# fulliu/lc

Measured on AMD Instinct MI355X. Metric: poses/sec (cov-loss fwd+bwd + weighted PnP), B=256 N=64, 1/2/4/8 MI355X, higher is better.
Workload: dtype f64; 1 GPU; configs[1]: synthetic B=256 N=64 2D-3D correspondences per GPU, HIP weighted-PnP + cov-loss; global_batch=256, n_points=64, launch=graph_region, launch_agreed_by_all_ranks=True

## Files before the change

### lc_amd/csrc/lc_common.h

```cpp
#pragma once
#include <hip/hip_runtime.h>

namespace lc {

#ifndef LC_NT_GRAD_STORES
#define LC_NT_GRAD_STORES 1
#endif
typedef float lc_v4f_t __attribute__((ext_vector_type(4)));
__device__ __forceinline__ void store_stream4(float* q, float a, float b, float c, float d) {
#if LC_NT_GRAD_STORES
    lc_v4f_t r = {a, b, c, d};
    __builtin_nontemporal_store(r, reinterpret_cast<lc_v4f_t*>(q));
#else
    *reinterpret_cast<float4*>(q) = make_float4(a, b, c, d);
#endif
}


constexpr int kWave = 64;

constexpr int kDppQuadXor1 = 0xB1;
constexpr int kDppQuadXor2 = 0x4E;
constexpr int kDppIdentity = 0xE4;
constexpr int kDppRowMirror = 0x140;
constexpr int kDppHalfMirror = 0x141;

template <int CTRL, int BANK_MASK = 0xF>
__device__ __forceinline__ double dpp_mov_f64(double old, double src) {
    const int lo = __builtin_amdgcn_update_dpp(__double2loint(old), __double2loint(src), CTRL, 0xF, BANK_MASK, false);
    const int hi = __builtin_amdgcn_update_dpp(__double2hiint(old), __double2hiint(src), CTRL, 0xF, BANK_MASK, false);
    return __hiloint2double(hi, lo);
}

__device__ __forceinline__ double shfl_f64(double v, int src) {
    const int lo = __shfl(__double2loint(v), src, kWave), hi = __shfl(__double2hiint(v), src, kWave);
    return __hiloint2double(hi, lo);
}

__device__ __forceinline__ double swap32_add(double a, double b) {
    const auto lo = __builtin_amdgcn_permlane32_swap(__double2loint(a), __double2loint(b), false, false);
    const auto hi = __builtin_amdgcn_permlane32_swap(__double2hiint(a), __double2hiint(b), false, false);
    return __hiloint2double(hi[0], lo[0]) + __hiloint2double(hi[1], lo[1]);
}
__device__ __forceinline__ double swap16_add(double a, double b) {
    const auto lo = __builtin_amdgcn_permlane16_swap(__double2loint(a), __double2loint(b), false, false);
    const auto hi = __builtin_amdgcn_permlane16_swap(__double2hiint(a), __double2hiint(b), false, false);
    return __hiloint2double(hi[0], lo[0]) + __hiloint2double(hi[1], lo[1]);
}

template <int CTRL, int BANK_UP>
__device__ __forceinline__ double dpp_exchange_add(double lo, double hi) {
    constexpr int BANK_DOWN = 0xF & ~BANK_UP;
    const double keep = dpp_mov_f64<kDppIdentity, BANK_UP>(lo, hi);
    double recv = dpp_mov_f64<CTRL, BANK_UP>(lo, hi);
    recv = dpp_mov_f64<CTRL, BANK_DOWN>(recv, lo);
    return keep + recv;
}

template <int K>
__device__ __forceinline__ void wave_allreduce(double (&v)[K]) {
#pragma unroll
    for (int i = 0; i < K; ++i) {
        double x = v[i];
        x += dpp_mov_f64<kDppQuadXor1>(x, x);
        x += dpp_mov_f64<kDppQuadXor2>(x, x);
        x += dpp_mov_f64<kDppHalfMirror>(x, x);
        x += dpp_mov_f64<kDppRowMirror>(x, x);
        x = swap16_add(x, x);
        x = swap32_add(x, x);
        v[i] = x;
    }
}

template <int K>
__device__ __forceinline__ void wave_reduce_scatter16(double (&v)[K], int ) {
    static_assert(K % 16 == 0, "K must be a multiple of 16");
    constexpr int R = K / 16;
#pragma unroll
    for (int i = 0; i < K / 2; ++i) v[i] = swap32_add(v[i], v[i + K / 2]);
#pragma unroll
    for (int i = 0; i < K / 4; ++i) v[i] = swap16_add(v[i], v[i + K / 4]);
#pragma unroll
    for (int i = 0; i < K / 8; ++i) v[i] = dpp_exchange_add<kDppRowMirror, 0xC>(v[i], v[i + K / 8]);
#pragma unroll
    for (int i = 0; i < K / 16; ++i) v[i] = dpp_exchange_add<kDppHalfMirror, 0xA>(v[i], v[i + K / 16]);
#pragma unroll
    for (int i = 0; i < R; ++i) {
        v[i] += dpp_mov_f64<kDppQuadXor2>(v[i], v[i]);
        v[i] += dpp_mov_f64<kDppQuadXor1>(v[i], v[i]);
    }
}

__device__ __forceinline__ int scatter16_base(int lane, int R) {
    return R * (((lane >> 5) & 1) * 8 + ((lane >> 4) & 1) * 4 + ((lane >> 3) & 1) * 2 + ((lane >> 2) & 1));
}

__device__ __forceinline__ double fast_rcp(double x) {
    const double y = __builtin_amdgcn_rcp(x);
    const double e = __builtin_fma(-x, y, 1.0);
    return __builtin_fma(y, e, y);
}

__device__ __forceinline__ void fast_sqrt_rsqrt(double x, double& s, double& rs) {
    const double r0 = __builtin_amdgcn_rsq(x);
    const double g = x * r0, h = 0.5 * r0;
    const double rr = __builtin_fma(-h, g, 0.5);
    const double g1 = __builtin_fma(g, rr, g), h1 = __builtin_fma(h, rr, h);
    s = x == 0.0 ? 0.0 : g1;
    rs = x == 0.0 ? r0 : 2.0 * h1;
}
__device__ __forceinline__ double fast_sqrt(double x) {
    double s, rs;
    fast_sqrt_rsqrt(x, s, rs);
    return s;
}

template <int NW>
constexpr int sum_bcast_lds_doubles(int K) { return K * 68 * NW + K; }

#ifndef LC_WAVE_SYNC
#define LC_WAVE_SYNC 0
#endif
__device__ __forceinline__ void wave_sync() {
    __builtin_amdgcn_fence(__ATOMIC_RELEASE, "wavefront");
    __builtin_amdgcn_wave_barrier();
    __builtin_amdgcn_fence(__ATOMIC_ACQUIRE, "wavefront");
}

template <class T>
__device__ __forceinline__ void xcd_store(T* q, T v) { __hip_atomic_store(q, v, __ATOMIC_RELAXED, __HIP_MEMORY_SCOPE_AGENT); }
template <class T>
__device__ __forceinline__ T xcd_load(const T* q) { return __hip_atomic_load(q, __ATOMIC_RELAXED, __HIP_MEMORY_SCOPE_AGENT); }
__device__ __forceinline__ void xcd_stores_done() { asm volatile("s_waitcnt vmcnt(0)" ::: "memory"); }

constexpr int kArrivalShards = 16, kArrivalStride = 32;
constexpr int kArrivalWords = (1 + kArrivalShards) * kArrivalStride;
__device__ __forceinline__ bool arrive_is_last(unsigned* words, unsigned block, unsigned blocks) {
    const unsigned shards = blocks < (unsigned)kArrivalShards ? blocks : (unsigned)kArrivalShards;
    const unsigned g = block % shards, members = (blocks - g + shards - 1) / shards;
    if (__hip_atomic_fetch_add(words + (1 + g) * kArrivalStride, 1u, __ATOMIC_RELAXED, __HIP_MEMORY_SCOPE_AGENT) != members - 1) return false;
    return __hip_atomic_fetch_add(words, 1u, __ATOMIC_RELAXED, __HIP_MEMORY_SCOPE_AGENT) == shards - 1;
}
__device__ __forceinline__ void arrival_reset(unsigned* words, int tid) {
    if (tid <= kArrivalShards) xcd_store(words + tid * kArrivalStride, 0u);
}

template <int NW>
__device__ __forceinline__ void block_sum_sync() {
    if constexpr (NW == 1 && !LC_WAVE_SYNC) wave_sync();
    else __syncthreads();
}

template <int NW>
__device__ __forceinline__ int block_sum_open(int tid) {
    block_sum_sync<NW>();
    return tid + 2 * (tid >> 5);
}
template <int NW>
__device__ __forceinline__ void block_sum_put(double* lds, int pos, int k, double v) { lds[k * (68 * NW) + pos] = v; }

template <int K, int NW>
__device__ __forceinline__ void block_sum_close(double (&v)[K], double* lds, int tid);

template <int K, int NW>
__device__ __forceinline__ void block_sum_bcast_lds(double (&v)[K], double* lds, int tid) {
    const int pos = block_sum_open<NW>(tid);
#pragma unroll
    for (int k = 0; k < K; ++k) block_sum_put<NW>(lds, pos, k, v[k]);
    block_sum_close<K, NW>(v, lds, tid);
}

template <int K, int NW>
__device__ __forceinline__ double* block_sum_totals(double* lds) { return lds + K * (68 * NW); }

template <int K, int NW>
__device__ __forceinline__ void block_sum_reduce(double* lds, int tid) {
    static_assert(K <= 32 && (NW == 1 || NW == 4), "unsupported shape");
    constexpr int LD = 68 * NW, S = 2 * NW;
    block_sum_sync<NW>();
    double s = 0;
    if (tid < K * S) {
        const double2* row = reinterpret_cast<const double2*>(lds + (tid / S) * LD + 34 * (tid % S));
        double2 a[8];
#pragma unroll
        for (int i = 0; i < 8; ++i) a[i] = row[i];
#pragma unroll
        for (int i = 0; i < 8; ++i) {
            const double2 t = row[8 + i];
            a[i].x += t.x;
            a[i].y += t.y;
        }
#pragma unroll
        for (int st = 4; st >= 1; st >>= 1) {
#pragma unroll
            for (int i = 0; i < st; ++i) { a[i].x += a[i + st].x; a[i].y += a[i + st].y; }
        }
        s = a[0].x + a[0].y;
    }
    s += dpp_mov_f64<kDppQuadXor1>(s, s);
    if constexpr (NW == 4) {
        s += dpp_mov_f64<kDppQuadXor2>(s, s);
        s += dpp_mov_f64<kDppHalfMirror>(s, s);
    }
    double* tot = lds + K * LD;
    if (tid < K * S && (tid % S) == 0) tot[tid / S] = s;
    block_sum_sync<NW>();
}

template <int K, int NW>
__device__ __forceinline__ void block_sum_close(double (&v)[K], double* lds, int tid) {
    block_sum_reduce<K, NW>(lds, tid);
    const double* tot = block_sum_totals<K, NW>(lds);
#pragma unroll
    for (int k = 0; k < K; ++k) v[k] = tot[k];
}

#ifndef LC_WIDE_SUM_REGS
#define LC_WIDE_SUM_REGS 1
#endif
template <int K>
__device__ __forceinline__ void block_sum_waves4(double (&v)[K], double* lds, int tid, int& phase) {
    static_assert(K <= 32, "one reduce-scatter of 32");
    const int lane = tid & 63, wave = tid >> 6;
    double w[32];
#pragma unroll
    for (int k = 0; k < 32; ++k) w[k] = k < K ? v[k] : 0.0;
    wave_reduce_scatter16<32>(w, lane);
    double* part = lds;
    double* tot = lds + 128 + 32 * phase;
    phase ^= 1;
    if ((lane & 3) == 0) *reinterpret_cast<double2*>(part + 32 * wave + scatter16_base(lane, 2)) = make_double2(w[0], w[1]);
    __syncthreads();
    if (tid < 32) tot[tid] = ((part[tid] + part[32 + tid]) + part[64 + tid]) + part[96 + tid];
    __syncthreads();
#pragma unroll
    for (int k = 0; k < K; ++k) v[k] = tot[k];
}

constexpr int kSplitMaxParts = 8;
#ifndef LC_SPLIT_WAIT_US
#define LC_SPLIT_WAIT_US 2000
#endif
constexpr unsigned long long kSplitWaitTicks = 100ull * LC_SPLIT_WAIT_US;
__device__ __forceinline__ bool split_wait_expired(int polls, unsigned long long& t0) {
    if ((polls & 15) != 15) return false;
    const unsigned long long now = __builtin_amdgcn_s_memrealtime();
    if (t0 == 0) { t0 = now; return false; }
    return now - t0 > kSplitWaitTicks;
}
constexpr int kSplitRowWords = 64;
constexpr size_t kSplitPoseBytes = 2 * kSplitMaxParts * kSplitRowWords * sizeof(unsigned long long) + 128;
constexpr int kSplitLdsDoubles = 128 + 64 + 2;
constexpr int kSplitSerialLdsDoubles = 128 + 32 * kSplitMaxParts + 32;
struct SplitSum {
    unsigned long long* exch;
    unsigned* epoch;
    int G, part;
    unsigned base;
    unsigned seq;
    bool timed_out;
};
__device__ __forceinline__ unsigned* split_tail(void* region, size_t region_bytes) {
    return reinterpret_cast<unsigned*>(static_cast<char*>(region) + region_bytes - 128);
}
__device__ __forceinline__ SplitSum split_sum_enter(void* pose_region, int G, int part) {
    unsigned* epoch = split_tail(pose_region, kSplitPoseBytes);
    return SplitSum{reinterpret_cast<unsigned long long*>(pose_region), epoch, G, part, xcd_load(epoch), 0u, false};
}
__device__ __forceinline__ void split_sum_leave(const SplitSum& sx) {
    if (sx.timed_out) xcd_store(sx.epoch + 1, 1u);
    else if (sx.part == 0 && sx.seq > 0) xcd_store(sx.epoch, sx.base + sx.seq);
}
__device__ __forceinline__ bool split_rescue_enter(void* region, size_t region_bytes, bool redo, int tid, int threads) {
    unsigned* tail = split_tail(region, region_bytes);
    const bool dirty = xcd_load(tail + 1) != 0u;
    if (!dirty && !redo) return false;
    __syncthreads();
    if (dirty) {
        unsigned long long* w = static_cast<unsigned long long*>(region);
        for (size_t i = tid; i < (region_bytes - 128) / 8; i += threads) xcd_store(w + i, 0ull);
        if (tid < 2) xcd_store(tail + tid, 0u);
    }
    if (redo && tid == 0) xcd_store(tail + 2, xcd_load(tail + 2) + 1u);
    return redo;
}

template <int K>
__device__ __forceinline__ void block_sum_split(double (&v)[K], double* lds, int tid, int& phase, SplitSum& sx) {
    static_assert(K <= 32, "one reduce-scatter of 32");
    const int lane = tid & 63, wave = tid >> 6;
    double w[32];
#pragma unroll
    for (int k = 0; k < 32; ++k) w[k] = k < K ? v[k] : 0.0;
    wave_reduce_scatter16<32>(w, lane);
    double* part = lds;
    double* tot = lds + 128 + 32 * phase;
    int* arrived_ok = reinterpret_cast<int*>(lds + 192);
    phase ^= 1;
    if (sx.timed_out) {
#pragma unroll
        for (int k = 0; k < K; ++k) v[k] = 0.0;
        return;
    }
    if ((lane & 3) == 0) *reinterpret_cast<double2*>(part + 32 * wave + scatter16_base(lane, 2)) = make_double2(w[0], w[1]);
    __syncthreads();
    if (tid < 32) {
        const unsigned long long ticket = (unsigned long long)(sx.base + sx.seq + 1u) << 32;
        unsigned long long* rows = sx.exch + (size_t)(sx.seq & 1u) * (kSplitMaxParts * kSplitRowWords) + 2 * tid;
        {
            const unsigned long long bits = __builtin_bit_cast(unsigned long long, ((part[tid] + part[32 + tid]) + part[64 + tid]) + part[96 + tid]);
            unsigned long long* mine = rows + sx.part * kSplitRowWords;
            xcd_store(mine, ticket | (bits & 0xFFFFFFFFull));
            xcd_store(mine + 1, ticket | (bits >> 32));
        }
        unsigned long long lo[kSplitMaxParts], hi[kSplitMaxParts];
        bool ok = true;
        unsigned long long t0 = 0;
        for (int polls = 0;; ++polls) {
#pragma unroll
            for (int g = 0; g < kSplitMaxParts; ++g)
                if (g < sx.G) {
                    lo[g] = xcd_load(rows + g * kSplitRowWords);
                    hi[g] = xcd_load(rows + g * kSplitRowWords + 1);
                }
            unsigned long long late = 0;
#pragma unroll
            for (int g = 0; g < kSplitMaxParts; ++g)
                if (g < sx.G) late |= ((lo[g] ^ ticket) | (hi[g] ^ ticket)) >> 32;
            if (late == 0) break;
            if (split_wait_expired(polls, t0)) { ok = false; break; }
            __builtin_amdgcn_s_sleep(1);
        }
        double s = 0.0;
#pragma unroll
        for (int g = 0; g < kSplitMaxParts; ++g)
            if (g < sx.G) s += __builtin_bit_cast(double, (hi[g] << 32) | (lo[g] & 0xFFFFFFFFull));
        tot[tid] = s;
        if (!ok) *arrived_ok = 0;
    }
    __syncthreads();
    if (!*arrived_ok) sx.timed_out = true;
#pragma unroll
    for (int k = 0; k < K; ++k) v[k] = tot[k];
    ++sx.seq;
}

template <int K>
__device__ __forceinline__ void block_sum_parts_serial(double (&v)[K], double* lds, int tid, int g, int G) {
    static_assert(K <= 32, "one reduce-scatter of 32");
    const int lane = tid & 63, wave = tid >> 6;
    double w[32];
#pragma unroll
    for (int k = 0; k < 32; ++k) w[k] = k < K ? v[k] : 0.0;
    wave_reduce_scatter16<32>(w, lane);
    double* part = lds;
    double* rows = lds + 128;
    double* tot = lds + 128 + 32 * kSplitMaxParts;
    if ((lane & 3) == 0) *reinterpret_cast<double2*>(part + 32 * wave + scatter16_base(lane, 2)) = make_double2(w[0], w[1]);
    __syncthreads();
    if (tid < 32) {
        rows[32 * g + tid] = ((part[tid] + part[32 + tid]) + part[64 + tid]) + part[96 + tid];
        if (g == G - 1) {
            double s = 0.0;
            for (int h = 0; h < G; ++h) s += rows[32 * h + tid];
            tot[tid] = s;
        }
    }
    __syncthreads();
    if (g == G - 1) {
#pragma unroll
        for (int k = 0; k < K; ++k) v[k] = tot[k];
    }
}

#ifndef LC_HORNER_ASM
#define LC_HORNER_ASM 1
#endif
__device__ __forceinline__ double horner_step(double p, double z, double c) {
#if LC_HORNER_ASM
    double r;
    asm("v_fma_f64 %0, %1, %2, %3" : "=v"(r) : "v"(p), "v"(z), "v"(c));
    return r;
#else
    return __builtin_fma(p, z, c);
#endif
}

__device__ __forceinline__ void sincos_small(double x, double& s, double& c) {
    if (!(x < 1.0e4)) {
        sincos(x, &s, &c);
        return;
    }
    const double kf = __builtin_rint(x * 0.63661977236758134308);
    const int q = (int)kf;
    double r = __builtin_fma(-kf, 1.57079632673412561417e+00, x);
    r = __builtin_fma(-kf, 6.07710050650619224932e-11, r);
    r = __builtin_fma(-kf, 2.02226624879595063154e-21, r);
    const double z = r * r;
    double ps = horner_step(1.58969099521155010221e-10, z, -2.50507602534068634195e-08);
    ps = horner_step(ps, z, 2.75573137070700676789e-06);
    ps = horner_step(ps, z, -1.98412698298579493134e-04);
    ps = horner_step(ps, z, 8.33333333332248946124e-03);
    ps = horner_step(ps, z, -1.66666666666666324348e-01);
    const double sr = __builtin_fma(ps * z, r, r);
    double pc = horner_step(-1.13596475577881948265e-11, z, 2.08757232129817482790e-09);
    pc = horner_step(pc, z, -2.75573143513906633035e-07);
    pc = horner_step(pc, z, 2.48015872894767294178e-05);
    pc = horner_step(pc, z, -1.38888888888741095749e-03);
    pc = horner_step(pc, z, 4.16666666666666019037e-02);
    const double cr = __builtin_fma(pc * z, z, __builtin_fma(-0.5, z, 1.0));
    const double ss = (q & 1) ? cr : sr, cc = (q & 1) ? sr : cr;
    s = (q & 2) ? -ss : ss;
    c = ((q + 1) & 2) ? -cc : cc;
}

__device__ __forceinline__ double atan_ratio_pos(double s, double c) {
    const bool swap = s > c;
    const double a = swap ? c : s, b = swap ? s : c;
    double t = a * fast_rcp(b);
#pragma unroll
    for (int k = 0; k < 2; ++k) {
        const double h = fast_sqrt(__builtin_fma(t, t, 1.0));
        t = t * fast_rcp(1.0 + h);
    }
    const double w = t * t;
    double p = horner_step(-1.0 / 21.0, w, 1.0 / 19.0);
    p = horner_step(p, w, -1.0 / 17.0);
    p = horner_step(p, w, 1.0 / 15.0);
    p = horner_step(p, w, -1.0 / 13.0);
    p = horner_step(p, w, 1.0 / 11.0);
    p = horner_step(p, w, -1.0 / 9.0);
    p = horner_step(p, w, 1.0 / 7.0);
    p = horner_step(p, w, -1.0 / 5.0);
    p = horner_step(p, w, 1.0 / 3.0);
    const double at = 4.0 * __builtin_fma(-(p * w), t, t);
    return swap ? 1.57079632679489661923 - at : at;
}

__device__ __forceinline__ bool uniform(bool c) { return __builtin_amdgcn_ballot_w64(c) != 0ull; }

__host__ __device__ constexpr int tri6(int i, int j) { return i * 6 - (i * (i - 1)) / 2 + (j - i); }

}
```

### lc_amd/csrc/lc_pnp_body.h

```cpp
#pragma once
#include <cfloat>

#include "lc_common.h"
#include "lc_kernels.h"

#ifdef LC_STAMPS
#define LC_PSTAMP_DECL unsigned long long pst_[8] = {0, 0, 0, 0, 0, 0, 0, 0}, pt0_ = 0, pt1_ = 0
#define LC_PSTAMP_BEGIN()                                                                 \
    do {                                                                                  \
        __builtin_amdgcn_sched_barrier(0);                                                \
        asm volatile("s_memtime %0\n\ts_waitcnt lgkmcnt(0)" : "=s"(pt0_)::"memory");      \
        __builtin_amdgcn_sched_barrier(0);                                                \
    } while (0)
#define LC_PSTAMP(i)                                                                      \
    do {                                                                                  \
        __builtin_amdgcn_sched_barrier(0);                                                \
        asm volatile("s_memtime %0\n\ts_waitcnt lgkmcnt(0)" : "=s"(pt1_)::"memory");      \
        __builtin_amdgcn_sched_barrier(0);                                                \
        pst_[i] += pt1_ - pt0_;                                                           \
        pt0_ = pt1_;                                                                      \
    } while (0)
#else
#define LC_PSTAMP_DECL
#define LC_PSTAMP_BEGIN() do {} while (0)
#define LC_PSTAMP(i) do {} while (0)
#endif

#ifndef LC_WIDE_REG_SUM_REGS
#define LC_WIDE_REG_SUM_REGS 1
#endif
#ifndef LC_PNP_STREAM_SUM
#define LC_PNP_STREAM_SUM 1
#endif

namespace lc {
namespace pnp {

template <int NW>
constexpr int kPnpLdsDoubles = sum_bcast_lds_doubles<NW>(28);

struct Point {
    double X[3];
    double u, v;
    double a, b, c;
};

struct Rot {
    double R[9];
    double Jr[9];
};

__device__ __forceinline__ void make_rot(const double aa[3], Rot& o) {
    const double x = aa[0], y = aa[1], z = aa[2];
    const double th2 = x * x + y * y + z * z;
    const bool small = !(th2 > DBL_EPSILON);
    double th, ith;
    fast_sqrt_rsqrt(th2, th, ith);
    double s, c;
    sincos_small(th, s, c);
    const double ith2 = ith * ith;
    const double A = small ? 1.0 : s * ith;
    const double B = small ? 0.0 : (1.0 - c) * ith2;
    const double C = small ? 0.0 : (th - s) * ith2 * ith;
    const double cd = small ? 1.0 : c;
    o.R[0] = cd + B * x * x;    o.R[1] = B * x * y - A * z; o.R[2] = B * x * z + A * y;
    o.R[3] = B * x * y + A * z; o.R[4] = cd + B * y * y;    o.R[5] = B * y * z - A * x;
    o.R[6] = B * x * z - A * y; o.R[7] = B * y * z + A * x; o.R[8] = cd + B * z * z;
    const double d = 1.0 - C * th2;
    o.Jr[0] = d + C * x * x;     o.Jr[1] = C * x * y + B * z; o.Jr[2] = C * x * z - B * y;
    o.Jr[3] = C * x * y - B * z; o.Jr[4] = d + C * y * y;     o.Jr[5] = C * y * z + B * x;
    o.Jr[6] = C * x * z + B * y; o.Jr[7] = C * y * z - B * x; o.Jr[8] = d + C * z * z;
}

template <bool FIRST, bool STREAM = false, int NW = 1>
__device__ __forceinline__ void accumulate_point(const Point& pt, const Rot& rt, const double t[3], const double k[6],
                                                 const double (&sc)[6], double (&acc)[28], double* lds = nullptr, int pos = 0) {
    double rx[3], q[3];
#pragma unroll
    for (int d = 0; d < 3; ++d) {
        rx[d] = rt.R[3 * d] * pt.X[0] + rt.R[3 * d + 1] * pt.X[1] + rt.R[3 * d + 2] * pt.X[2];
        q[d] = rx[d] + t[d];
    }
    const double iz = fast_rcp(q[2]);
    const double up = (q[0] * k[0] + q[1] * k[1]) * iz, vp = (q[0] * k[3] + q[1] * k[4]) * iz;
    const double du = up - pt.u, dv = vp - pt.v;
    const double r[2] = {du * pt.a + dv * pt.b, dv * pt.c};
    const double dup[3] = {k[0] * iz, k[1] * iz, -up * iz};
    const double dvp[3] = {k[3] * iz, k[4] * iz, -vp * iz};
    double J[2][6];
#pragma unroll
    for (int m = 0; m < 3; ++m) {
        J[0][3 + m] = pt.a * dup[m] + pt.b * dvp[m];
        J[1][3 + m] = pt.c * dvp[m];
    }
#pragma unroll
    for (int rr = 0; rr < 2; ++rr) {
        double cr[3];
        cr[0] = rx[1] * J[rr][5] - rx[2] * J[rr][4];
        cr[1] = rx[2] * J[rr][3] - rx[0] * J[rr][5];
        cr[2] = rx[0] * J[rr][4] - rx[1] * J[rr][3];
#pragma unroll
        for (int m = 0; m < 3; ++m) J[rr][m] = (rt.Jr[3 * m] * cr[0] + rt.Jr[3 * m + 1] * cr[1] + rt.Jr[3 * m + 2] * cr[2]) * sc[m];
#pragma unroll
        for (int m = 0; m < 3; ++m) J[rr][3 + m] *= sc[3 + m];
    }
#pragma unroll
    for (int i = 0; i < 6; ++i) {
#pragma unroll
        for (int j = i; j < 6; ++j) {
            const double v = __builtin_fma(J[0][i], J[0][j], J[1][i] * J[1][j]);
            if constexpr (STREAM) block_sum_put<NW>(lds, pos, tri6(i, j), v);
            else acc[tri6(i, j)] = FIRST ? v : acc[tri6(i, j)] + v;
        }
        const double gi = __builtin_fma(J[0][i], r[0], J[1][i] * r[1]);
        if constexpr (STREAM) block_sum_put<NW>(lds, pos, 21 + i, gi);
        else acc[21 + i] = FIRST ? gi : acc[21 + i] + gi;
    }
    const double ss = __builtin_fma(r[0], r[0], r[1] * r[1]);
    if constexpr (STREAM) block_sum_put<NW>(lds, pos, 27, ss);
    else acc[27] = FIRST ? ss : acc[27] + ss;
}

__device__ __forceinline__ bool ldlt_solve6(const double (&A)[21], const double (&dg)[6], const double (&rhs)[6], double (&y)[6]) {
    double L[6][6], Ld[6][6], id[6];
    bool ok = true;
#pragma unroll
    for (int j = 0; j < 6; ++j) {
        double dj = A[tri6(j, j)] + dg[j];
#pragma unroll
        for (int k = 0; k < j; ++k) dj -= L[j][k] * Ld[j][k];
        ok = ok && (dj > 0) && (dj < DBL_MAX);
        id[j] = fast_rcp(dj);
#pragma unroll
        for (int i = j + 1; i < 6; ++i) {
            double v = A[tri6(j, i)];
#pragma unroll
            for (int k = 0; k < j; ++k) v -= L[i][k] * Ld[j][k];
            Ld[i][j] = v;
            L[i][j] = v * id[j];
        }
    }
    double z[6];
#pragma unroll
    for (int i = 0; i < 6; ++i) {
        double v = rhs[i];
#pragma unroll
        for (int k = 0; k < i; ++k) v -= L[i][k] * z[k];
        z[i] = v;
    }
#pragma unroll
    for (int i = 5; i >= 0; --i) {
        double v = z[i] * id[i];
#pragma unroll
        for (int k = i + 1; k < 6; ++k) v -= L[k][i] * y[k];
        y[i] = v;
    }
    return ok;
}

struct RawPoint {
    float X[3];
    float2 u;
    float a, b, c;
};
__device__ __forceinline__ float nan_to_num(float f) { return f != f ? 0.f : fminf(fmaxf(f, -FLT_MAX), FLT_MAX); }

template <bool OPTS = false>
__device__ __forceinline__ RawPoint load_raw_point(const PnpParams& p, size_t base, int n) {
    RawPoint o;
    const float* X = p.pts3d + (base + n) * 3;
    o.u = *reinterpret_cast<const float2*>(p.pts2d + (base + n) * 2);
    o.X[0] = X[0]; o.X[1] = X[1]; o.X[2] = X[2];
    if (OPTS && p.weight_mask) {
        const float m = p.weight_mask[base + n] ? 1.f : 0.f;
        o.a = m; o.b = 0.f; o.c = m;
    } else if (p.sqrtL) {
        const float4 L = *reinterpret_cast<const float4*>(p.sqrtL + (base + n) * 4);
        o.a = L.x; o.b = L.z; o.c = L.w;
    } else {
        const float2 L = *reinterpret_cast<const float2*>(p.sqrt_diag + (base + n) * 2);
        o.a = L.x; o.b = 0.f; o.c = L.y;
    }
    if constexpr (OPTS) {
        if (p.options & kPnpWeightsAreStd) { o.a = 1.f / (o.a * o.a); o.c = 1.f / (o.c * o.c); }
        if (p.options & kPnpNanToNum) {
            o.u.x = nan_to_num(o.u.x); o.u.y = nan_to_num(o.u.y);
            o.X[0] = nan_to_num(o.X[0]); o.X[1] = nan_to_num(o.X[1]); o.X[2] = nan_to_num(o.X[2]);
            o.a = nan_to_num(o.a); o.b = nan_to_num(o.b); o.c = nan_to_num(o.c);
        }
        if (p.options & kPnpWeightsAreIcov) { o.a = sqrtf(o.a); o.c = sqrtf(o.c); }
    }
    return o;
}
__device__ __forceinline__ Point to_point(const RawPoint& r, const double cam[6]) {
    Point o;
    o.X[0] = r.X[0]; o.X[1] = r.X[1]; o.X[2] = r.X[2];
    o.u = (double)r.u.x - cam[2];
    o.v = (double)r.u.y - cam[5];
    o.a = r.a; o.b = r.b; o.c = r.c;
    return o;
}
template <bool OPTS = false>
__device__ __forceinline__ Point load_point(const PnpParams& p, size_t base, int n, const double cam[6]) {
    return to_point(load_raw_point<OPTS>(p, base, n), cam);
}

__device__ __forceinline__ double max_abs6(const double (&v)[6]) {
    double m = 0;
#pragma unroll
    for (int j = 0; j < 6; ++j) m = fmax(m, fabs(v[j]));
    return m;
}
__device__ __forceinline__ double norm6(const double (&v)[6]) {
    double m = 0;
#pragma unroll
    for (int j = 0; j < 6; ++j) m += v[j] * v[j];
    return fast_sqrt(m);
}

template <bool REG, int NW = 1, bool TRACE = false, bool OPTS = false, int PPT = 0, bool TAIL = false, int SPLIT = 0>
__device__ __forceinline__ void solve_pose(const PnpParams& p, int b, int lane, double* bc, bool store = true, float* handoff = nullptr,
                                           const float* start_override = nullptr, [[maybe_unused]] SplitSum* sx = nullptr) {
    constexpr int kThreads = kWave * NW;
    static_assert(SPLIT != 1 || (NW == 4 && !REG && PPT > 0 && !TRACE), "the split form is the four-wave cached-prefix solve");
    static_assert(SPLIT != 2 || (NW == 4 && !REG && PPT == 0 && !TRACE), "the rescue form walks memory, part by part");
    const int slot = SPLIT == 1 ? lane + kThreads * sx->part : lane;
    const int stride = SPLIT == 1 ? kThreads * sx->G : kThreads;
#ifdef LC_TRACE_CLOCK
    const unsigned long long t_start_ = __builtin_amdgcn_s_memtime();
#endif
    LC_PSTAMP_DECL;
    LC_PSTAMP_BEGIN();
    const int n = p.counts ? p.counts[b] : p.Nmax;
    const int bk = (OPTS && p.pose_mod > 0) ? b % p.pose_mod : b;
    const float* st_in = start_override ? start_override : (p.start ? p.start + 7 * (size_t)bk : p.states + 7 * (size_t)b);
    const bool filter = OPTS && (p.options & kPnpNanToNum);
    auto fin = [&](float f) { return filter ? nan_to_num(f) : f; };
    if (n < 3) {
        if (lane == 0 && store) {
            p.rets[b] = 1;
            p.result_tr[b] = 1.f;
            if (p.iters) p.iters[b] = 0;
        }
        if (lane < 7) {
            const float v = fin(st_in[lane]);
            if (store && (p.start || start_override || filter)) p.states[7 * (size_t)b + lane] = v;
            if (handoff) handoff[lane] = v;
        }
        return;
    }
    const size_t base = (size_t)b * p.Nmax;
    const bool active = lane < n;
    RawPoint raw;
    if constexpr (REG) raw = load_raw_point<OPTS>(p, base, active ? lane : 0);
    [[maybe_unused]] RawPoint rawc[PPT > 0 ? PPT : 1];
    if constexpr (!REG && PPT > 0) {
#pragma unroll
        for (int k = 0; k < PPT; ++k)
            if (slot + k * stride < n) rawc[k] = load_raw_point<OPTS>(p, base, slot + k * stride);
    }
    double cam[6];
    {
        const float* Kp = p.K + 9 * (size_t)bk;
#pragma unroll
        for (int i = 0; i < 6; ++i) cam[i] = fin(Kp[i]);
    }
    double x[6];
    {
        float stf[7];
#pragma unroll
        for (int i = 0; i < 7; ++i) stf[i] = st_in[i];
        asm volatile("" : "+v"(stf[0]), "+v"(stf[1]), "+v"(stf[2]), "+v"(stf[3]), "+v"(stf[4]), "+v"(stf[5]), "+v"(stf[6]));
        const double q0 = fin(stf[0]), q1 = fin(stf[1]), q2 = fin(stf[2]), q3 = fin(stf[3]);
        const double s2 = q1 * q1 + q2 * q2 + q3 * q3;
        double kk = 2.0;
        if (s2 > 0.0) {
            const double s = fast_sqrt(s2);
            const double half = atan_ratio_pos(s, fabs(q0));
            const double two_theta = 2.0 * ((q0 < 0.0) ? -half : half);
            kk = two_theta / s;
        }
        x[0] = q1 * kk; x[1] = q2 * kk; x[2] = q3 * kk;
        x[3] = fin(stf[4]); x[4] = fin(stf[5]); x[5] = fin(stf[6]);
    }
    LC_PSTAMP(0);
    Point rp;
    if constexpr (REG) {
        rp = to_point(raw, cam);
        if (!active) { rp.a = 0.0; rp.b = 0.0; rp.c = 0.0; }
    }

    [[maybe_unused]] int sum_phase = 0;
    auto evaluate = [&](const double (&xe)[6], const double (&sc)[6], double (&H)[21], double (&g)[6], double& cost) -> bool {
        LC_PSTAMP(1);
        Rot rt;
        make_rot(xe, rt);
        LC_PSTAMP(2);
        const double t[3] = {xe[3], xe[4], xe[5]};
        double acc[28];
        if constexpr (REG && LC_PNP_STREAM_SUM && !(NW == 4 && LC_WIDE_REG_SUM_REGS)) {
            const int pos = block_sum_open<NW>(lane);
            accumulate_point<true, true, NW>(rp, rt, t, cam, sc, acc, bc, pos);
            LC_PSTAMP(3);
            block_sum_close<28, NW>(acc, bc, lane);
        } else if constexpr (REG) {
            accumulate_point<true>(rp, rt, t, cam, sc, acc);
            LC_PSTAMP(3);
            if constexpr (NW == 4 && LC_WIDE_SUM_REGS) block_sum_waves4<28>(acc, bc, lane, sum_phase);
            else block_sum_bcast_lds<28, NW>(acc, bc, lane);
        } else {
#pragma unroll
            for (int i = 0; i < 28; ++i) acc[i] = 0;
            if constexpr (PPT > 0) {
#pragma unroll
                for (int k = 0; k < PPT; ++k)
                    if (slot + k * stride < n) accumulate_point<false>(to_point(rawc[k], cam), rt, t, cam, sc, acc);
                if constexpr (TAIL)
                    for (int i = slot + PPT * stride; i < n; i += stride) accumulate_point<false>(load_point<OPTS>(p, base, i, cam), rt, t, cam, sc, acc);
            } else if constexpr (SPLIT == 2) {
                for (int g = 0; g < sx->G; ++g) {
                    if (g > 0) {
#pragma unroll
                        for (int i = 0; i < 28; ++i) acc[i] = 0;
                    }
                    for (int i = lane + kThreads * g; i < n; i += kThreads * sx->G) accumulate_point<false>(load_point<OPTS>(p, base, i, cam), rt, t, cam, sc, acc);
                    block_sum_parts_serial<28>(acc, bc, lane, g, sx->G);
                }
            } else {
                for (int i = lane; i < n; i += kThreads) accumulate_point<false>(load_point<OPTS>(p, base, i, cam), rt, t, cam, sc, acc);
            }
            LC_PSTAMP(3);
            if constexpr (SPLIT == 2) {}
            else if constexpr (SPLIT == 1) block_sum_split<28>(acc, bc, lane, sum_phase, *sx);
            else if constexpr (NW == 4 && LC_WIDE_SUM_REGS) block_sum_waves4<28>(acc, bc, lane, sum_phase);
            else block_sum_bcast_lds<28, NW>(acc, bc, lane);
        }
        LC_PSTAMP(4);
#pragma unroll
        for (int i = 0; i < 21; ++i) H[i] = acc[i];
#pragma unroll
        for (int i = 0; i < 6; ++i) g[i] = acc[21 + i];
        const double ss = acc[27];
        cost = 0.5 * ss;
        double chk = ss;
#pragma unroll
        for (int i = 0; i < 6; ++i) chk += H[tri6(i, i)];
        LC_PSTAMP(5);
        if constexpr (SPLIT == 1) {
            if (sx->timed_out) return false;
        }
        return chk <= DBL_MAX;
    };

    const double ftol = p.ftol, ptol = 1e-8, gtol = 1e-10;
    double H[21], g[6], cost;
    double scale[6], iscale[6];
    bool failed;
    {
        const double one[6] = {1, 1, 1, 1, 1, 1};
        failed = !evaluate(x, one, H, g, cost);
#pragma unroll
        for (int j = 0; j < 6; ++j) {
            iscale[j] = 1.0 + fast_sqrt(H[tri6(j, j)]);
            scale[j] = fast_rcp(iscale[j]);
        }
#pragma unroll
        for (int i = 0; i < 6; ++i) {
#pragma unroll
            for (int j = i; j < 6; ++j) H[tri6(i, j)] *= scale[i] * scale[j];
            g[i] *= scale[i];
        }
    }
    auto grad_max = [&](const double (&gs)[6]) {
        double m = 0;
#pragma unroll
        for (int j = 0; j < 6; ++j) m = fmax(m, fabs(gs[j]) * iscale[j]);
        return m;
    };
    double gmax = grad_max(g);
    auto sqnorm6 = [](const double (&v)[6]) {
        double m = 0;
#pragma unroll
        for (int j = 0; j < 6; ++j) m += v[j] * v[j];
        return m;
    };
    double xn2 = sqnorm6(x);
    double radius = 1e4, dfac = 2.0;
    int iter = 0, n_invalid = 0;
    bool converged = false;
    auto trace = [&](int kind, double cost_x, double cost_cand, double mcc, double rho, double step_norm) {
        if constexpr (TRACE) {
            if (lane == 0 && p.trace && iter <= p.trace_rows) {
                double* row = p.trace + ((size_t)b * p.trace_rows + (iter - 1)) * 8;
                row[0] = kind; row[1] = cost_x; row[2] = cost_cand; row[3] = mcc; row[4] = rho; row[5] = step_norm;
                row[6] = radius; row[7] = gmax;
#ifdef LC_TRACE_CLOCK
                row[7] = (double)(__builtin_amdgcn_s_memtime() - t_start_);
#endif
            }
        }
    };

    while (uniform(!failed && !converged)) {
        if (iter >= p.max_iter) break;
        if (uniform(gmax <= gtol || radius <= 1e-32)) { converged = true; break; }
        ++iter;
        double dg[6], y[6];
        const double inv_radius = fast_rcp(radius);
#pragma unroll
        for (int i = 0; i < 6; ++i) dg[i] = fmin(fmax(H[tri6(i, i)], 1e-6), 1e32) * inv_radius;
        LC_PSTAMP(1);
        bool step_ok = ldlt_solve6(H, dg, g, y);
        LC_PSTAMP(6);
        double mcc = 0;
#pragma unroll
        for (int i = 0; i < 6; ++i) mcc += y[i] * (g[i] + dg[i] * y[i]);
        mcc *= 0.5;
        step_ok = step_ok && (mcc > 0.0) && (mcc <= DBL_MAX);
        if (uniform(!step_ok)) {
            if (++n_invalid >= 5) { failed = true; trace(0, cost, 0.0, mcc, 0.0, 0.0); break; }
            radius /= dfac; dfac *= 2.0;
            trace(0, cost, 0.0, mcc, 0.0, 0.0);
            continue;
        }
        n_invalid = 0;
        double xc[6], delta[6];
#pragma unroll
        for (int j = 0; j < 6; ++j) { delta[j] = -y[j] * scale[j]; xc[j] = x[j] + delta[j]; }
        const double sn2 = sqnorm6(delta);
        const bool ptol_in_reach = TRACE || uniform(!(sn2 > 2.0 * ptol * ptol * (xn2 + ptol * ptol)));
        double step_norm = 0.0;
        bool ptol_hit = false;
        if (ptol_in_reach) {
            step_norm = fast_sqrt(sn2);
            ptol_hit = uniform(step_norm <= ptol * (fast_sqrt(xn2) + ptol));
        }
        double cost_c;
        const bool cand_ok = evaluate(xc, scale, H, g, cost_c);
        if constexpr (SPLIT == 1) {
            if (sx->timed_out) { failed = true; break; }
        }
        if (!cand_ok) cost_c = DBL_MAX;
        if (ptol_hit) {
            converged = true; trace(3, cost, cost_c, mcc, 0.0, step_norm); break;
        }
        const double cost_change = cost - cost_c;
        if (uniform(fabs(cost_change) <= ftol * cost)) {
            converged = true; trace(4, cost, cost_c, mcc, cost_change * fast_rcp(mcc), step_norm); break;
        }
        const double rel = cost_change * fast_rcp(mcc);
        if (uniform(rel > 1e-3)) {
#pragma unroll
            for (int j = 0; j < 6; ++j) x[j] = xc[j];
            const double cost_prev = cost;
            cost = cost_c;
            xn2 = sqnorm6(x);
            gmax = grad_max(g);
            const double tq = 2.0 * rel - 1.0;
            radius = fmin(1e16, radius * fast_rcp(fmax(1.0 / 3.0, 1.0 - tq * tq * tq)));
            dfac = 2.0;
            trace(1, cost_prev, cost_c, mcc, rel, step_norm);
        } else {
            radius /= dfac; dfac *= 2.0;
            trace(2, cost, cost_c, mcc, rel, step_norm);
            double cost_again;
            if (!evaluate(x, scale, H, g, cost_again)) { failed = true; break; }
        }
    }
    LC_PSTAMP(1);
#ifdef LC_STAMPS
    if (lane == 0 && p.iters) {
        unsigned long long* o = reinterpret_cast<unsigned long long*>(p.iters) + 8 * (size_t)b;
        for (int i = 0; i < 6; ++i) o[i] = pst_[i];
        o[6] = iter;
        o[7] = pst_[6];
    }
#endif
    const bool invalid = failed || !converged;
    if (invalid && lane < 7) {
        const float v = fin(st_in[lane]);
        if (store && (p.start || start_override || filter)) p.states[7 * (size_t)b + lane] = v;
        if (handoff) handoff[lane] = v;
    }
    if (lane == 0) {
        if (store) {
            p.rets[b] = invalid ? 1 : 0;
            if constexpr (SPLIT == 1) {
                if (sx->timed_out) p.rets[b] = kPnpPartNeverArrived;
            }
            p.result_tr[b] = (float)radius;
#ifndef LC_STAMPS
            if (p.iters) p.iters[b] = iter;
#endif
        }
        if (!invalid) {
            float stq[7];
            float* st = stq;
            const double t2 = x[0] * x[0] + x[1] * x[1] + x[2] * x[2];
            double q0 = 1.0, kk = 0.5;
            if (t2 > 0.0) {
                const double th = fast_sqrt(t2), h = 0.5 * th;
                double sh, ch;
                sincos_small(h, sh, ch);
                q0 = ch;
                kk = sh / th;
            }
            st[0] = (float)q0; st[1] = (float)(x[0] * kk); st[2] = (float)(x[1] * kk); st[3] = (float)(x[2] * kk);
            st[4] = (float)x[3]; st[5] = (float)x[4]; st[6] = (float)x[5];
#pragma unroll
            for (int k = 0; k < 7; ++k) {
                if (store) p.states[7 * (size_t)b + k] = stq[k];
                if (handoff) handoff[k] = stq[k];
            }
        }
    }
}


constexpr int kPnpLowregLdsDoubles = kPnpLdsDoubles<1> + 30;

__device__ __forceinline__ bool ldlt_solve6_lds(const double* A, const double* g, double inv_radius, double (&y)[6], double& mcc) {
    double L[6][6], Ld[6][6], id[6];
    bool ok = true;
    auto dgv = [&](int i) { return fmin(fmax(A[tri6(i, i)], 1e-6), 1e32) * inv_radius; };
#pragma unroll
    for (int j = 0; j < 6; ++j) {
        double dj = A[tri6(j, j)] + dgv(j);
#pragma unroll
        for (int k = 0; k < j; ++k) dj -= L[j][k] * Ld[j][k];
        ok = ok && (dj > 0) && (dj < DBL_MAX);
        id[j] = fast_rcp(dj);
#pragma unroll
        for (int i = j + 1; i < 6; ++i) {
            double v = A[tri6(j, i)];
#pragma unroll
            for (int k = 0; k < j; ++k) v -= L[i][k] * Ld[j][k];
            Ld[i][j] = v;
            L[i][j] = v * id[j];
        }
    }
    double z[6];
#pragma unroll
    for (int i = 0; i < 6; ++i) {
        double v = g[i];
#pragma unroll
        for (int k = 0; k < i; ++k) v -= L[i][k] * z[k];
        z[i] = v;
    }
#pragma unroll
    for (int i = 5; i >= 0; --i) {
        double v = z[i] * id[i];
#pragma unroll
        for (int k = i + 1; k < 6; ++k) v -= L[k][i] * y[k];
        y[i] = v;
    }
    mcc = 0;
#pragma unroll
    for (int i = 0; i < 6; ++i) mcc += y[i] * (g[i] + dgv(i) * y[i]);
    mcc *= 0.5;
    return ok;
}

template <bool OPTS = false>
__device__ __forceinline__ void solve_pose_lowreg(const PnpParams& p, int b, int lane, double* bc) {
    const int n = p.counts ? p.counts[b] : p.Nmax;
    const int bk = (OPTS && p.pose_mod > 0) ? b % p.pose_mod : b;
    const float* st_in = (p.start ? p.start + 7 * (size_t)bk : p.states + 7 * (size_t)b);
    const bool filter = OPTS && (p.options & kPnpNanToNum);
    auto fin = [&](float f) { return filter ? nan_to_num(f) : f; };
    if (n < 3) {
        if (lane == 0) {
            p.rets[b] = 1;
            p.result_tr[b] = 1.f;
            if (p.iters) p.iters[b] = 0;
        }
        if ((p.start || filter) && lane < 7) p.states[7 * (size_t)b + lane] = fin(st_in[lane]);
        return;
    }
    const size_t base = (size_t)b * p.Nmax;
    const bool active = lane < n;
    const RawPoint raw = load_raw_point<OPTS>(p, base, active ? lane : 0);
    double cam[6];
    {
        const float* Kp = p.K + 9 * (size_t)bk;
#pragma unroll
        for (int i = 0; i < 6; ++i) cam[i] = fin(Kp[i]);
    }
    double* const tot = block_sum_totals<28, 1>(bc);
    double* const ux = bc + kPnpLdsDoubles<1>;
    double* const uscale = ux + 6;
    double* const uiscale = ux + 12;
    double* const uxc = ux + 18;
    double* const ucam = ux + 24;
    if (lane == 0) {
#pragma unroll
        for (int i = 0; i < 6; ++i) ucam[i] = cam[i];
    }
    {
        double x[6];
        const double q0 = fin(st_in[0]), q1 = fin(st_in[1]), q2 = fin(st_in[2]), q3 = fin(st_in[3]);
        const double s2 = q1 * q1 + q2 * q2 + q3 * q3;
        double kk = 2.0;
        if (s2 > 0.0) {
            const double s = fast_sqrt(s2);
            const double half = atan_ratio_pos(s, fabs(q0));
            const double two_theta = 2.0 * ((q0 < 0.0) ? -half : half);
            kk = two_theta / s;
        }
        x[0] = q1 * kk; x[1] = q2 * kk; x[2] = q3 * kk;
        x[3] = fin(st_in[4]); x[4] = fin(st_in[5]); x[5] = fin(st_in[6]);
        if (lane == 0) {
#pragma unroll
            for (int j = 0; j < 6; ++j) { ux[j] = x[j]; uscale[j] = 1.0; }
        }
        wave_sync();
    }
    Point rp = to_point(raw, cam);
    if (!active) { rp.a = 0.0; rp.b = 0.0; rp.c = 0.0; }

    auto evaluate = [&](const double* xe, double& cost) -> bool {
        double xv[6], sc[6];
#pragma unroll
        for (int j = 0; j < 6; ++j) { xv[j] = xe[j]; sc[j] = uscale[j]; }
        Rot rt;
        make_rot(xv, rt);
        const double t[3] = {xv[3], xv[4], xv[5]};
        double acc[28];
        const int pos = block_sum_open<1>(lane);
        accumulate_point<true, true, 1>(rp, rt, t, ucam, sc, acc, bc, pos);
        block_sum_reduce<28, 1>(bc, lane);
        const double ss = tot[27];
        cost = 0.5 * ss;
        double chk = ss;
#pragma unroll
        for (int i = 0; i < 6; ++i) chk += tot[tri6(i, i)];
        return chk <= DBL_MAX;
    };

    const double ftol = p.ftol, ptol = 1e-8, gtol = 1e-10;
    double cost;
    bool failed = !evaluate(ux, cost);
    {
        double scale[6], iscale[6];
#pragma unroll
        for (int j = 0; j < 6; ++j) {
            iscale[j] = 1.0 + fast_sqrt(tot[tri6(j, j)]);
            scale[j] = fast_rcp(iscale[j]);
        }
        double Hs[21], gs[6];
#pragma unroll
        for (int i = 0; i < 6; ++i) {
#pragma unroll
            for (int j = i; j < 6; ++j) { double h = tot[tri6(i, j)]; h *= scale[i] * scale[j]; Hs[tri6(i, j)] = h; }
            double gi = tot[21 + i]; gi *= scale[i]; gs[i] = gi;
        }
        wave_sync();
        if (lane == 0) {
#pragma unroll
            for (int k = 0; k < 21; ++k) tot[k] = Hs[k];
#pragma unroll
            for (int j = 0; j < 6; ++j) { tot[21 + j] = gs[j]; uscale[j] = scale[j]; uiscale[j] = iscale[j]; }
        }
        wave_sync();
    }
    auto grad_max = [&]() {
        double m = 0;
#pragma unroll
        for (int j = 0; j < 6; ++j) m = fmax(m, fabs(tot[21 + j]) * uiscale[j]);
        return m;
    };
    auto sqnorm6 = [](const double* v) {
        double m = 0;
#pragma unroll
        for (int j = 0; j < 6; ++j) m += v[j] * v[j];
        return m;
    };
    double gmax = grad_max();
    double xn2 = sqnorm6(ux);
    double radius = 1e4, dfac = 2.0;
    int iter = 0, n_invalid = 0;
    bool converged = false;

    while (uniform(!failed && !converged)) {
        if (iter >= p.max_iter) break;
        if (uniform(gmax <= gtol || radius <= 1e-32)) { converged = true; break; }
        ++iter;
        double y[6], mcc;
        const double inv_radius = fast_rcp(radius);
        bool step_ok = ldlt_solve6_lds(tot, tot + 21, inv_radius, y, mcc);
        step_ok = step_ok && (mcc > 0.0) && (mcc <= DBL_MAX);
        if (uniform(!step_ok)) {
            if (++n_invalid >= 5) { failed = true; break; }
            radius /= dfac; dfac *= 2.0;
            continue;
        }
        n_invalid = 0;
        double sn2;
        {
            double xc[6], delta[6];
#pragma unroll
            for (int j = 0; j < 6; ++j) { delta[j] = -y[j] * uscale[j]; xc[j] = ux[j] + delta[j]; }
            sn2 = 0;
#pragma unroll
            for (int j = 0; j < 6; ++j) sn2 += delta[j] * delta[j];
            if (lane == 0) {
#pragma unroll
                for (int j = 0; j < 6; ++j) uxc[j] = xc[j];
            }
            wave_sync();
        }
        const bool ptol_in_reach = uniform(!(sn2 > 2.0 * ptol * ptol * (xn2 + ptol * ptol)));
        bool ptol_hit = false;
        if (ptol_in_reach) ptol_hit = uniform(fast_sqrt(sn2) <= ptol * (fast_sqrt(xn2) + ptol));
        double cost_c;
        const bool cand_ok = evaluate(uxc, cost_c);
        if (!cand_ok) cost_c = DBL_MAX;
        if (ptol_hit) { converged = true; break; }
        const double cost_change = cost - cost_c;
        if (uniform(fabs(cost_change) <= ftol * cost)) { converged = true; break; }
        const double rel = cost_change * fast_rcp(mcc);
        if (uniform(rel > 1e-3)) {
            double xn[6];
#pragma unroll
            for (int j = 0; j < 6; ++j) xn[j] = uxc[j];
            wave_sync();
            if (lane == 0) {
#pragma unroll
                for (int j = 0; j < 6; ++j) ux[j] = xn[j];
            }
            wave_sync();
            cost = cost_c;
            xn2 = sqnorm6(ux);
            gmax = grad_max();
            const double tq = 2.0 * rel - 1.0;
            radius = fmin(1e16, radius * fast_rcp(fmax(1.0 / 3.0, 1.0 - tq * tq * tq)));
            dfac = 2.0;
        } else {
            radius /= dfac; dfac *= 2.0;
            double cost_again;
            if (!evaluate(ux, cost_again)) { failed = true; break; }
        }
    }
    const bool invalid = failed || !converged;
    if (invalid && (p.start || filter) && lane < 7) p.states[7 * (size_t)b + lane] = fin(st_in[lane]);
    if (lane == 0) {
        p.rets[b] = invalid ? 1 : 0;
        p.result_tr[b] = (float)radius;
        if (p.iters) p.iters[b] = iter;
        if (!invalid) {
            float* st = p.states + 7 * (size_t)b;
            double x[6];
#pragma unroll
            for (int j = 0; j < 6; ++j) x[j] = ux[j];
            const double t2 = x[0] * x[0] + x[1] * x[1] + x[2] * x[2];
            double q0 = 1.0, kk = 0.5;
            if (t2 > 0.0) {
                const double th = fast_sqrt(t2), h = 0.5 * th;
                double sh, ch;
                sincos_small(h, sh, ch);
                q0 = ch;
                kk = sh / th;
            }
            st[0] = (float)q0; st[1] = (float)(x[0] * kk); st[2] = (float)(x[1] * kk); st[3] = (float)(x[2] * kk);
            st[4] = (float)x[3]; st[5] = (float)x[4]; st[6] = (float)x[5];
        }
    }
}

}
}
```

Before: 19.83 million poses/s.

## Add cost-only evaluation to skip Jacobian/Hessian build on terminal LM iteration

When the predicted cost change is within the ftol band, the solver first evaluates only the residual cost of the candidate, without the rotation Jacobian or the Hessian/gradient accumulation. If that cost meets the ftol convergence test (with a small safety band), it exits the loop without the full evaluate call. This is meant to avoid the 28-term block reduction and Jacobian math on the final iteration. The price is an extra cost-only pass and reduction whenever the prediction misses, and it adds a float-based finiteness guard that may differ slightly from the full path's check.

```diff
diff --git a/lc_amd/csrc/lc_common.h b/lc_amd/csrc/lc_common.h
--- a/lc_amd/csrc/lc_common.h
+++ b/lc_amd/csrc/lc_common.h
@@ -215,6 +215,14 @@
     for (int k = 0; k < K; ++k) v[k] = tot[k];
 }
 
+template <int ROW, int NW>
+__device__ __forceinline__ double block_sum_row(double v, double* lds, int tid) {
+    double* row = lds + ROW * (68 * NW);
+    row[block_sum_open<NW>(tid)] = v;
+    block_sum_reduce<1, NW>(row, tid);
+    return block_sum_totals<1, NW>(row)[0];
+}
+
 #ifndef LC_WIDE_SUM_REGS
 #define LC_WIDE_SUM_REGS 1
 #endif
@@ -235,6 +243,21 @@
     __syncthreads();
 #pragma unroll
     for (int k = 0; k < K; ++k) v[k] = tot[k];
+}
+
+template <int ROW>
+__device__ __forceinline__ double block_sum_waves4_row(double v, double* lds, int tid, int& phase) {
+    const int lane = tid & 63, wave = tid >> 6;
+    double w[1] = {v};
+    wave_allreduce<1>(w);
+    double* part = lds;
+    double* tot = lds + 128 + 32 * phase;
+    phase ^= 1;
+    if (lane == 0) part[32 * wave + ROW] = w[0];
+    __syncthreads();
+    if (tid == 0) tot[ROW] = ((part[ROW] + part[32 + ROW]) + part[64 + ROW]) + part[96 + ROW];
+    __syncthreads();
+    return tot[ROW];
 }
 
 constexpr int kSplitMaxParts = 8;
diff --git a/lc_amd/csrc/lc_pnp_body.h b/lc_amd/csrc/lc_pnp_body.h
--- a/lc_amd/csrc/lc_pnp_body.h
+++ b/lc_amd/csrc/lc_pnp_body.h
@@ -32,9 +32,22 @@
 #ifndef LC_PNP_STREAM_SUM
 #define LC_PNP_STREAM_SUM 1
 #endif
+#ifndef LC_PNP_TERMINAL_COST_ONLY
+#define LC_PNP_TERMINAL_COST_ONLY 1
+#endif
+
+#ifndef LC_PNP_TERMINAL_SUM_DPP
+#define LC_PNP_TERMINAL_SUM_DPP 0
+#endif
 
 namespace lc {
 namespace pnp {
+
+#ifndef LC_PNP_TERMINAL_PREDICT
+#define LC_PNP_TERMINAL_PREDICT 1.0
+#endif
+constexpr double kTerminalPredict = LC_PNP_TERMINAL_PREDICT;
+constexpr double kTerminalBand = 1e-10;
 
 template <int NW>
 constexpr int kPnpLdsDoubles = sum_bcast_lds_doubles<NW>(28);
@@ -50,6 +63,7 @@
     double Jr[9];
 };
 
+template <bool WITH_JR = true>
 __device__ __forceinline__ void make_rot(const double aa[3], Rot& o) {
     const double x = aa[0], y = aa[1], z = aa[2];
     const double th2 = x * x + y * y + z * z;
@@ -61,30 +75,49 @@
     const double ith2 = ith * ith;
     const double A = small ? 1.0 : s * ith;
     const double B = small ? 0.0 : (1.0 - c) * ith2;
-    const double C = small ? 0.0 : (th - s) * ith2 * ith;
+    [[maybe_unused]] const double C = small ? 0.0 : (th - s) * ith2 * ith;
     const double cd = small ? 1.0 : c;
     o.R[0] = cd + B * x * x;    o.R[1] = B * x * y - A * z; o.R[2] = B * x * z + A * y;
     o.R[3] = B * x * y + A * z; o.R[4] = cd + B * y * y;    o.R[5] = B * y * z - A * x;
     o.R[6] = B * x * z - A * y; o.R[7] = B * y * z + A * x; o.R[8] = cd + B * z * z;
-    const double d = 1.0 - C * th2;
-    o.Jr[0] = d + C * x * x;     o.Jr[1] = C * x * y + B * z; o.Jr[2] = C * x * z - B * y;
-    o.Jr[3] = C * x * y - B * z; o.Jr[4] = d + C * y * y;     o.Jr[5] = C * y * z + B * x;
-    o.Jr[6] = C * x * z + B * y; o.Jr[7] = C * y * z - B * x; o.Jr[8] = d + C * z * z;
+    if constexpr (WITH_JR) {
+        const double d = 1.0 - C * th2;
+        o.Jr[0] = d + C * x * x;     o.Jr[1] = C * x * y + B * z; o.Jr[2] = C * x * z - B * y;
+        o.Jr[3] = C * x * y - B * z; o.Jr[4] = d + C * y * y;     o.Jr[5] = C * y * z + B * x;
+        o.Jr[6] = C * x * z + B * y; o.Jr[7] = C * y * z - B * x; o.Jr[8] = d + C * z * z;
+    }
+}
+
+__device__ __forceinline__ void project_residual(const Point& pt, const double (&R)[9], const double t[3], const double k[6],
+                                                 double (&rx)[3], double& iz, double& up, double& vp, double (&r)[2]) {
+    double q[3];
+#pragma unroll
+    for (int d = 0; d < 3; ++d) {
+        rx[d] = R[3 * d] * pt.X[0] + R[3 * d + 1] * pt.X[1] + R[3 * d + 2] * pt.X[2];
+        q[d] = rx[d] + t[d];
+    }
+    iz = fast_rcp(q[2]);
+    up = (q[0] * k[0] + q[1] * k[1]) * iz;
+    vp = (q[0] * k[3] + q[1] * k[4]) * iz;
+    const double du = up - pt.u, dv = vp - pt.v;
+    r[0] = du * pt.a + dv * pt.b;
+    r[1] = dv * pt.c;
+}
+
+__device__ __forceinline__ double point_cost(const Point& pt, const double (&R)[9], const double t[3], const double k[6], double kabs) {
+    double rx[3], iz, up, vp, r[2];
+    project_residual(pt, R, t, k, rx, iz, up, vp, r);
+    const double ss = __builtin_fma(r[0], r[0], r[1] * r[1]);
+    const float jb = (fabsf((float)pt.a) + fabsf((float)pt.b) + fabsf((float)pt.c)) * fabsf((float)iz) * ((float)kabs + fabsf((float)up) + fabsf((float)vp)) *
+                     (1.f + fabsf((float)rx[0]) + fabsf((float)rx[1]) + fabsf((float)rx[2]));
+    return jb < 1e18f ? ss : __builtin_inf();
 }
 
 template <bool FIRST, bool STREAM = false, int NW = 1>
 __device__ __forceinline__ void accumulate_point(const Point& pt, const Rot& rt, const double t[3], const double k[6],
                                                  const double (&sc)[6], double (&acc)[28], double* lds = nullptr, int pos = 0) {
-    double rx[3], q[3];
-#pragma unroll
-    for (int d = 0; d < 3; ++d) {
-        rx[d] = rt.R[3 * d] * pt.X[0] + rt.R[3 * d + 1] * pt.X[1] + rt.R[3 * d + 2] * pt.X[2];
-        q[d] = rx[d] + t[d];
-    }
-    const double iz = fast_rcp(q[2]);
-    const double up = (q[0] * k[0] + q[1] * k[1]) * iz, vp = (q[0] * k[3] + q[1] * k[4]) * iz;
-    const double du = up - pt.u, dv = vp - pt.v;
-    const double r[2] = {du * pt.a + dv * pt.b, dv * pt.c};
+    double rx[3], iz, up, vp, r[2];
+    project_residual(pt, rt.R, t, k, rx, iz, up, vp, r);
     const double dup[3] = {k[0] * iz, k[1] * iz, -up * iz};
     const double dvp[3] = {k[3] * iz, k[4] * iz, -vp * iz};
     double J[2][6];
@@ -352,6 +385,40 @@
         return chk <= DBL_MAX;
     };
 
+    [[maybe_unused]] auto evaluate_cost = [&](const double (&xe)[6], double& cost) -> bool {
+        LC_PSTAMP(1);
+        Rot rt;
+        make_rot<false>(xe, rt);
+        LC_PSTAMP(2);
+        const double t[3] = {xe[3], xe[4], xe[5]};
+        const double kabs = fabs(cam[0]) + fabs(cam[1]) + fabs(cam[3]) + fabs(cam[4]);
+        double ss;
+        if constexpr (REG) {
+            ss = point_cost(rp, rt.R, t, cam, kabs);
+        } else {
+            ss = 0;
+            if constexpr (PPT > 0) {
+#pragma unroll
+                for (int k = 0; k < PPT; ++k)
+                    if (slot + k * stride < n) ss += point_cost(to_point(rawc[k], cam), rt.R, t, cam, kabs);
+                if constexpr (TAIL)
+                    for (int i = slot + PPT * stride; i < n; i += stride) ss += point_cost(load_point<OPTS>(p, base, i, cam), rt.R, t, cam, kabs);
+            } else {
+                for (int i = lane; i < n; i += kThreads) ss += point_cost(load_point<OPTS>(p, base, i, cam), rt.R, t, cam, kabs);
+            }
+        }
+        LC_PSTAMP(3);
+        if constexpr (NW == 1 && LC_PNP_TERMINAL_SUM_DPP) {
+            double w[1] = {ss};
+            wave_allreduce<1>(w);
+            ss = w[0];
+        } else if constexpr (NW == 4 && LC_WIDE_SUM_REGS && !(REG && LC_PNP_STREAM_SUM && !LC_WIDE_REG_SUM_REGS)) ss = block_sum_waves4_row<27>(ss, bc, lane, sum_phase);
+        else ss = block_sum_row<27, NW>(ss, bc, lane);
+        LC_PSTAMP(4);
+        cost = 0.5 * ss;
+        return ss <= DBL_MAX;
+    };
+
     const double ftol = p.ftol, ptol = 1e-8, gtol = 1e-10;
     double H[21], g[6], cost;
     double scale[6], iscale[6];
@@ -388,6 +455,8 @@
     double radius = 1e4, dfac = 2.0;
     int iter = 0, n_invalid = 0;
     bool converged = false;
+    constexpr bool kTerminalCostOnly = LC_PNP_TERMINAL_COST_ONLY && !TRACE && SPLIT == 0 && !(NW == 4 && (REG || TAIL));
+    [[maybe_unused]] const bool terminal_in_reach = p.ftol <= 1.f && n <= (1 << 18);
     auto trace = [&](int kind, double cost_x, double cost_cand, double mcc, double rho, double step_norm) {
         if constexpr (TRACE) {
             if (lane == 0 && p.trace && iter <= p.trace_rows) {
@@ -434,6 +503,14 @@
         if (ptol_in_reach) {
             step_norm = fast_sqrt(sn2);
             ptol_hit = uniform(step_norm <= ptol * (fast_sqrt(xn2) + ptol));
+        }
+        if constexpr (kTerminalCostOnly) {
+            if (ptol_hit) { converged = true; break; }
+            if (uniform(mcc <= kTerminalPredict * ftol * cost) && terminal_in_reach) {
+                double cost_only;
+                const bool finite = evaluate_cost(xc, cost_only);
+                if (uniform(finite && fabs(cost - cost_only) <= ftol * cost - kTerminalBand * cost)) { converged = true; break; }
+            }
         }
         double cost_c;
         const bool cand_ok = evaluate(xc, scale, H, g, cost_c);
```

New measurement: 19.36 million poses/s. 0.976x the previous value.
